# google/hdrnet

Measured on NVIDIA H100. Metric: megapixels/s BilateralSliceApply @4K, higher is better.
Workload: dtype f32

## Files before the change

### hdrnet_b200/csrc/common.cuh

```cuda
#pragma once

#include <cuda_runtime.h>
#include <stdint.h>

#include "hdrnet_b200.h"

namespace hdrnet_b200 {

struct SliceGeom {
  int B;
  int H;
  int W;
  int rows;
  int y_off;
  int gh, gw, gd;
  float scale_x;
  float scale_y;
};

__host__ inline SliceGeom make_geom(int B, int H, int W, int rows, int y_off, int gh, int gw,
                                    int gd) {
  SliceGeom g;
  g.B = B; g.H = H; g.W = W; g.rows = rows; g.y_off = y_off;
  g.gh = gh; g.gw = gw; g.gd = gd;
// ... 131 lines not shown
               "r"(smem_u32(smem_src)), "r"(bytes)
               : "memory");
}
__device__ __forceinline__ void tma_store_commit() {
  asm volatile("cp.async.bulk.commit_group;" ::: "memory");
}
template <int N>
__device__ __forceinline__ void tma_store_wait_read() {
  asm volatile("cp.async.bulk.wait_group.read %0;" ::"n"(N) : "memory");
}
template <int N>
__device__ __forceinline__ void tma_store_wait_all() {
  asm volatile("cp.async.bulk.wait_group %0;" ::"n"(N) : "memory");
}
__device__ __forceinline__ void l2_prefetch_bulk(const void* gmem_src, uint32_t bytes) {
  asm volatile("cp.async.bulk.prefetch.L2.global [%0], %1;" ::"l"(gmem_src), "r"(bytes) : "memory");
}
__device__ __forceinline__ void fence_proxy_async_smem() {
  asm volatile("fence.proxy.async.shared::cta;" ::: "memory");
}

__device__ __forceinline__ uint64_t l2_policy_evict_first() {
  uint64_t p;
  asm volatile("createpolicy.fractional.L2::evict_first.b64 %0, 1.0;" : "=l"(p));
  return p;
}
__device__ __forceinline__ uint64_t l2_policy_evict_last() {
  uint64_t p;
  asm volatile("createpolicy.fractional.L2::evict_last.b64 %0, 1.0;" : "=l"(p));
  return p;
}
__device__ __forceinline__ void tma_load_1d(void* smem_dst, const void* gmem_src, uint32_t bytes,
                                            uint64_t* bar, uint64_t policy) {
  asm volatile(
      "cp.async.bulk.shared::cluster.global.mbarrier::complete_tx::bytes.L2::cache_hint"
      " [%0], [%1], %2, [%3], %4;"
      ::"r"(smem_u32(smem_dst)), "l"(gmem_src), "r"(bytes), "r"(smem_u32(bar)), "l"(policy)
      : "memory");
}
__device__ __forceinline__ void tma_store_1d(void* gmem_dst, const void* smem_src, uint32_t bytes,
                                             uint64_t policy) {
  asm volatile("cp.async.bulk.global.shared::cta.bulk_group.L2::cache_hint [%0], [%1], %2, %3;"
               ::"l"(gmem_dst), "r"(smem_u32(smem_src)), "r"(bytes), "l"(policy)
               : "memory");
}
__device__ __forceinline__ void st_global_hint(float4* p, const float4& v, uint64_t policy) {
  asm volatile("st.global.L2::cache_hint.v4.f32 [%0], {%1, %2, %3, %4}, %5;"
               ::"l"(p), "f"(v.x), "f"(v.y), "f"(v.z), "f"(v.w), "l"(policy)
               : "memory");
}
__device__ __forceinline__ void l2_discard_line(const void* p) {
  asm volatile("discard.global.L2 [%0], 128;" ::"l"(p) : "memory");
}

}
```

### hdrnet_b200/csrc/slice_apply.cu

```cuda
#include <cuda_runtime.h>

#include <atomic>

#include <algorithm>
#include <climits>
#include <cstdint>
#include <cstdlib>
#include <mutex>
#include <new>
#include <vector>

#include "slice_rows.cuh"

namespace hdrnet_b200 {


template <bool kApply>
__global__ void __launch_bounds__(256)
slice_generic_kernel(const float* __restrict__ grid, const float* __restrict__ guide,
                     const float* __restrict__ input, float* __restrict__ out, SliceGeom g,
                     int n_in, int n_out, int J, long long npix) {
  const int gc = kApply ? n_out * J : J;
  const long long grid_image = static_cast<long long>(g.gh) * g.gw * g.gd * gc;
  const long long stride = static_cast<long long>(gridDim.x) * blockDim.x;
// ... 602 lines not shown
      ws[static_cast<size_t>(row) * n_out + e] = lerp4(1.0f - ay.f, va, ay.f, vb);
    }
  }
}

static int launch_yblend(const float* grid, float* ws, const SliceGeom& g, int row_floats, cudaStream_t stream) {
  const long long total_rows = static_cast<long long>(g.B) * g.rows;
  const unsigned blocks = static_cast<unsigned>((total_rows + kYblendRows - 1) / kYblendRows);
  yblend_rows_kernel<<<blocks, 256, 0, stream>>>(grid, reinterpret_cast<float4*>(ws), g, row_floats);
  return static_cast<int>(cudaGetLastError());
}


static int device_sm_count() {
  int dev = 0, sms = 0;
  if (cudaGetDevice(&dev) != cudaSuccess) return 132;
  if (cudaDeviceGetAttribute(&sms, cudaDevAttrMultiProcessorCount, dev) != cudaSuccess) return 132;
  return sms > 0 ? sms : 132;
}

static int device_max_smem_optin() {
  int dev = 0, v = 0;
  if (cudaGetDevice(&dev) != cudaSuccess) return 227 * 1024;
  if (cudaDeviceGetAttribute(&v, cudaDevAttrMaxSharedMemoryPerBlockOptin, dev) != cudaSuccess)
    return 227 * 1024;
  return v;
}

static int device_texture_alignment() {
  int dev = 0, v = 0;
  if (cudaGetDevice(&dev) != cudaSuccess) return 512;
  if (cudaDeviceGetAttribute(&v, cudaDevAttrTextureAlignment, dev) != cudaSuccess) return 512;
  return v > 0 ? v : 512;
}


static bool make_tma_plan(const SliceGeom& g, int max_smem, int sms, TmaPlan* out, bool tex_mode,
                          int threads, int in_fmt = kPxF32, int out_fmt = kPxF32, int grid_rows = 0) {
  const int in_bpp = 3 * px_bytes_per_channel(in_fmt), out_bpp = 3 * px_bytes_per_channel(out_fmt);
  const int gran = std::max(4, std::max(16 / std::__gcd(16, in_bpp), 16 / std::__gcd(16, out_bpp)));
  if (g.W < gran || (g.W % gran) != 0) return false;
  TmaPlan p;
  p.threads = threads;
  p.row_floats = g.gw * g.gd * kGc;
  p.in_bpp = in_bpp;
  p.out_bpp = out_bpp;
  const int quads = g.W / 4;
  p.nseg = (quads + threads - 1) / threads;
  p.seg_px = round_up(4 * ((quads + p.nseg - 1) / p.nseg), gran);
  p.off_guide = round_up(p.seg_px * in_bpp, 16);
  p.off_out = (out_bpp == in_bpp) ? 0 : p.off_guide + p.seg_px * 4;
  p.stage_bytes = round_up((p.off_out ? p.off_out + p.seg_px * out_bpp : p.off_guide + p.seg_px * 4), 128);
  p.off_raw = 256;
  p.off_slab = p.off_raw + round_up(2 * p.row_floats * 4, 128);
  p.off_grid = p.off_slab;
  p.off_stage = p.off_slab + (tex_mode ? grid_rows * round_up(p.row_floats * 4, 128) : round_up(p.row_floats * 4, 128));
  const int per_cta_2 = (max_smem + 1024) / 2 - 1024;
  int stages = 0, resident = 0;
  for (int ns = 4; ns >= 2 && stages == 0; --ns)
    if (p.off_stage + ns * p.stage_bytes <= per_cta_2) { stages = ns; resident = 2; }
  for (int ns = 4; ns >= 2 && stages == 0; --ns)
    if (p.off_stage + ns * p.stage_bytes <= max_smem) { stages = ns; resident = 1; }
  if (stages == 0) return false;
  p.stages = stages;
  p.resident = resident;
  p.smem_bytes = p.off_stage + stages * p.stage_bytes;
  const long long total_rows = static_cast<long long>(g.B) * g.rows;
  p.ctas = static_cast<int>(std::min<long long>(total_rows, static_cast<long long>(sms) * resident));
  *out = p;
  return true;
}

static inline bool aligned16(const void* p) { return (reinterpret_cast<uintptr_t>(p) & 15u) == 0; }

static int validate_common(int B, int H, int W, int gh, int gw, int gd) {
  if (B < 0 || H < 0 || W < 0) return HDRNET_E_BAD_SHAPE;
  if (gh < 1 || gw < 1 || gd < 1) return HDRNET_E_BAD_SHAPE;
  return HDRNET_OK;
}

static int generic_grid(long long npix, int sms) {
  const long long blocks = (npix + 255) / 256;
  return static_cast<int>(std::min<long long>(blocks, static_cast<long long>(sms) * 16));
}

template <class GuideFn, int kTexChunks = 0, int kMinBlocks = 2, int kThreads = kTmaThreads,
          int kIn = kPxF32, int kOut = kPxF32>
static int launch_tma_occ(const TmaArgs& a, const GuideFn& fn, cudaStream_t stream) {
  auto kern = slice_apply_rows_tma_kernel<GuideFn, kTexChunks, kMinBlocks, kThreads, kIn, kOut>;
  cudaError_t e = cudaFuncSetAttribute(kern, cudaFuncAttributeMaxDynamicSharedMemorySize,
                                       a.p.smem_bytes);
  if (e != cudaSuccess) return static_cast<int>(e);
  kern<<<a.p.ctas, kThreads, a.p.smem_bytes, stream>>>(a, fn);
  return static_cast<int>(cudaGetLastError());
}

template <class GuideFn, int kTexChunks = 0>
static int launch_tma(const TmaArgs& a, const GuideFn& fn, cudaStream_t stream, int in_fmt = kPxF32,
                      int out_fmt = kPxF32) {
  if constexpr (GuideFn::kFromInput) {
    if constexpr (kTexChunks > 0) return launch_tma_occ<GuideFn, kTexChunks, 2, kTexThreads>(a, fn, stream);
    else return launch_tma_occ<GuideFn, 0, 2>(a, fn, stream);
  } else {
    if (in_fmt == kPxU8 && out_fmt == kPxU8)
      return launch_tma_occ<GuideFn, kTexChunks, 2, kTmaThreads, kPxU8, kPxU8>(a, fn, stream);
    if (in_fmt == kPxU16 && out_fmt == kPxU8)
// ... 113 lines not shown

static int graph_slab_texture(const float* ws, size_t bytes, cudaGraph_t graph, cudaTextureObject_t* out) {
  cudaStreamCaptureMode mode = cudaStreamCaptureModeRelaxed;
  cudaError_t err = cudaThreadExchangeStreamCaptureMode(&mode);
  if (err != cudaSuccess) { (void)cudaGetLastError(); return static_cast<int>(err); }
  const int rc = graph_slab_texture_relaxed(ws, bytes, graph, out);
  cudaThreadExchangeStreamCaptureMode(&mode);
  return rc;
}

struct GuideSpec {
  int mode;
  const float* guide;
  float* guide_out;
  const CurvesGuideParams* curves;
  const NNGuideParams* nn;
  float* workspace = nullptr;
  size_t workspace_bytes = 0;
  int in_fmt = kPxF32;
  int out_fmt = kPxF32;
};


template <class GuideFn>
static int launch_px_generic(const float* grid, const void* input, void* out, float* guide_out,
                             const SliceGeom& g, long long npix, int blocks, int in_fmt, int out_fmt,
                             const GuideFn& fn, cudaStream_t stream) {
  const unsigned char* in = static_cast<const unsigned char*>(input);
  unsigned char* o = static_cast<unsigned char*>(out);
#define HDRNET_PX_CASE(I, O)                                                                    \
  if (in_fmt == I && out_fmt == O) {                                                            \
    slice_apply_px_generic_kernel<GuideFn, I, O><<<blocks, 256, 0, stream>>>(grid, in, o,       \
                                                                           guide_out, g, npix, fn); \
    return static_cast<int>(cudaGetLastError());                                                \
  }
  HDRNET_PX_CASE(kPxU8, kPxU8)
  HDRNET_PX_CASE(kPxU16, kPxU8)
  HDRNET_PX_CASE(kPxF32, kPxU8)
  HDRNET_PX_CASE(kPxU8, kPxF32)
  HDRNET_PX_CASE(kPxU16, kPxF32)
  HDRNET_PX_CASE(kPxU8, kPxU16)
  HDRNET_PX_CASE(kPxU16, kPxU16)
  HDRNET_PX_CASE(kPxF32, kPxU16)
#undef HDRNET_PX_CASE
  return HDRNET_E_UNSUPPORTED;
}

struct ApplyForm {
  int variant;
  TmaPlan p;
  bool pre_pass;
  bool slab_warp;
  bool lean;
  bool fused_async;
  bool rows_any;
  int ctas, threads;
  size_t smem_bytes;
};

static int plan_slice_apply(const SliceGeom& g, int n_in, int n_out, int has_offset, int mode, int in_fmt,
                            int out_fmt, bool aligned, uintptr_t ws_base, size_t ws_bytes, int variant,
                            ApplyForm* f) {
  const int sms = device_sm_count();
  const int max_smem = device_max_smem_optin();
  const bool px = in_fmt != kPxF32 || out_fmt != kPxF32;
  const long long npix = static_cast<long long>(g.B) * g.rows * g.W;
  *f = ApplyForm{};

  TmaPlan plan;
  const bool row_shape = n_in == 3 && n_out == 3 && has_offset && aligned &&
                         (!px || (in_fmt != kPxF32 && (out_fmt == kPxU8 || out_fmt == kPxU16))) &&
                         make_tma_plan(g, max_smem, sms, &plan, false, kTmaThreads, in_fmt, out_fmt);
  const bool tex_ok = row_shape && ws_base != 0 && ws_base % device_texture_alignment() == 0 &&
                      ws_bytes >= static_cast<size_t>(g.B) * g.rows * plan.row_floats * sizeof(float) &&
                      ws_bytes / 16 <= (1u << 27);
  TmaPlan aplan, splan;
  const bool async_ok = tex_ok && mode == 0 && !px &&
                        make_tma_plan(g, max_smem, sms, &aplan, true, kAsyncThreads - 32) &&
                        aplan.resident == 2 && aplan.seg_px <= aplan.threads * 4;
  const bool slab_lines = (static_cast<size_t>(plan.row_floats) * sizeof(float)) % 128 == 0 && ws_base % 128 == 0;
  const bool slab_warp = async_ok && slab_lines &&
                         make_tma_plan(g, max_smem, sms, &splan, true, kAsyncThreads - 32, kPxF32, kPxF32, 2) &&
                         splan.resident == 2 && splan.seg_px <= splan.threads * 4 &&
                         splan.stages >= kAsyncAutoMinStages;

  const bool auto_req = variant == HDRNET_VARIANT_AUTO;
  if (auto_req) {
    if (tex_ok && g.W >= 128 && npix >= (1LL << 21))
      variant = (async_ok && aplan.stages >= kAsyncAutoMinStages) ? HDRNET_VARIANT_TEX_ASYNC : HDRNET_VARIANT_TEX;
    else
      variant = (row_shape && g.W >= 128) ? HDRNET_VARIANT_TMA : HDRNET_VARIANT_GENERIC;
  }
  f->variant = variant;

  if (variant == HDRNET_VARIANT_GENERIC) {
    if (mode != 0 && !px) return HDRNET_E_UNSUPPORTED;
    const int J = n_in + (has_offset ? 1 : 0);
    const AnyArgs aa{nullptr, nullptr, nullptr, nullptr, g, n_in, n_out, J, n_out * J, g.gw * g.gd * n_out * J};
    const size_t smem = (auto_req && mode == 0) ? rows_any_smem(aa, true, max_smem) : 0;
    f->rows_any = smem != 0;
    f->ctas = f->rows_any ? rows_any_ctas(g, sms) : generic_grid(npix, sms);
    f->threads = f->rows_any ? kAnyThreads : 256;
    f->smem_bytes = smem;
    return HDRNET_OK;
  }
  if (variant == HDRNET_VARIANT_TMA) {
    if (!row_shape) return HDRNET_E_UNSUPPORTED;
    f->p = plan;
  } else if (variant == HDRNET_VARIANT_TEX_ASYNC) {
    if (!async_ok) return HDRNET_E_UNSUPPORTED;
    f->slab_warp = slab_warp;
    f->pre_pass = !slab_warp;
    f->lean = static_cast<long long>(g.W) >= 4LL * g.gw;
    f->p = slab_warp ? splan : aplan;
  } else {
    if (!tex_ok) return HDRNET_E_UNSUPPORTED;
    f->pre_pass = true;
    TmaPlan fplan;
    f->fused_async = mode == 1 &&
                     make_tma_plan(g, max_smem, sms, &fplan, true, kFusedAsyncMathThreads, in_fmt, out_fmt) &&
                     fplan.resident == kFusedAsyncResident && fplan.stages >= 3;
    if (f->fused_async) {
      f->p = fplan;
    } else if (!make_tma_plan(g, max_smem, sms, &f->p, true, mode != 0 ? kTmaThreads : kTexThreads, in_fmt, out_fmt)) {
      return HDRNET_E_UNSUPPORTED;
    }
  }
  const bool issuer = variant == HDRNET_VARIANT_TEX_ASYNC || f->fused_async;
  f->ctas = f->p.ctas;
  f->threads = f->p.threads + (issuer ? 32 : 0) + (f->slab_warp ? 32 : 0);
  f->smem_bytes = f->p.smem_bytes;
  return HDRNET_OK;
}

template <int kTexChunks>
static int launch_block_sync(const TmaArgs& a, const GuideSpec& gs, cudaStream_t stream) {
  if (gs.mode == 1) { GuideCurves fn; fn.p = *gs.curves; return launch_tma<GuideCurves, kTexChunks>(a, fn, stream, gs.in_fmt, gs.out_fmt); }
  if (gs.mode == 2 && gs.nn->feats <= 16) {
    GuideNN<16> fn; fn.p = *gs.nn;
    return launch_tma<GuideNN<16>, kTexChunks>(a, fn, stream, gs.in_fmt, gs.out_fmt);
  }
  if (gs.mode == 2) {
    GuideNN<kMaxGuideFeats> fn; fn.p = *gs.nn;
    return launch_tma<GuideNN<kMaxGuideFeats>, kTexChunks>(a, fn, stream, gs.in_fmt, gs.out_fmt);
  }
  return launch_tma<GuideFromInput, kTexChunks>(a, GuideFromInput{}, stream);
}

static int launch_slice_apply_impl(const float* grid, const GuideSpec& gs, const void* input_v,
                                   void* out_v, int B, int H, int W, int rows, int y_off, int gh,
                                   int gw, int gd, int n_in, int n_out, int has_offset,
                                   int variant, cudaStream_t stream) {
  const float* input = static_cast<const float*>(input_v);
  float* out = static_cast<float*>(out_v);
  const bool px = gs.in_fmt != kPxF32 || gs.out_fmt != kPxF32;
  if (px) {
    if (gs.mode == 0 || n_in != 3 || n_out != 3 || !has_offset) return HDRNET_E_UNSUPPORTED;
    if (gs.in_fmt < kPxF32 || gs.in_fmt > kPxU16 || gs.out_fmt < kPxF32 || gs.out_fmt > kPxU16)
      return HDRNET_E_UNSUPPORTED;
  }
  int rc = validate_common(B, H, W, gh, gw, gd);
  if (rc != HDRNET_OK) return rc;
  if (n_in < 1 || n_out < 1 || rows < 0 || y_off < 0 || y_off + rows > H) return HDRNET_E_BAD_SHAPE;
  const long long npix = static_cast<long long>(B) * rows * W;
  if (npix == 0) return HDRNET_OK;
  if (!grid || !input || !out || (gs.mode == 0 && !gs.guide)) return HDRNET_E_NULL_POINTER;
  if (gs.out_fmt == kPxU16) {
    const uintptr_t o0 = reinterpret_cast<uintptr_t>(out_v), o1 = o0 + static_cast<uintptr_t>(npix) * 6u;
    const uintptr_t i0 = reinterpret_cast<uintptr_t>(input_v),
                    i1 = i0 + static_cast<uintptr_t>(npix) * 3u * px_bytes_per_channel(gs.in_fmt);
    const uintptr_t g0 = reinterpret_cast<uintptr_t>(grid),
                    g1 = g0 + static_cast<uintptr_t>(B) * gh * gw * gd * kGc * sizeof(float);
    if ((o0 < i1 && i0 < o1) || (o0 < g1 && g0 < o1)) return HDRNET_E_UNSUPPORTED;
  }
  const int J = n_in + (has_offset ? 1 : 0);
  const long long grid_floats = static_cast<long long>(gh) * gw * gd * n_out * J;
  if (grid_floats > INT_MAX || static_cast<long long>(rows) * B > INT_MAX / 4) return HDRNET_E_TOO_LARGE;
  if (variant != HDRNET_VARIANT_AUTO && variant != HDRNET_VARIANT_GENERIC && variant != HDRNET_VARIANT_TMA &&
      variant != HDRNET_VARIANT_TEX && variant != HDRNET_VARIANT_TEX_ASYNC)
    return HDRNET_E_UNSUPPORTED;

  const SliceGeom g = make_geom(B, H, W, rows, y_off, gh, gw, gd);
  const bool aligned = aligned16(grid) && aligned16(input) && aligned16(out) &&
                       (gs.mode != 0 || aligned16(gs.guide)) && (gs.guide_out == nullptr || aligned16(gs.guide_out));
  ApplyForm f;
  rc = plan_slice_apply(g, n_in, n_out, has_offset, gs.mode, gs.in_fmt, gs.out_fmt, aligned,
                        reinterpret_cast<uintptr_t>(gs.workspace), gs.workspace_bytes, variant, &f);
  if (rc != HDRNET_OK) return rc;

  if (f.variant == HDRNET_VARIANT_GENERIC) {
    if (px) {
      if (gs.mode == 1) { GuideCurves fn; fn.p = *gs.curves;
                          return launch_px_generic(grid, input_v, out_v, gs.guide_out, g, npix, f.ctas, gs.in_fmt, gs.out_fmt, fn, stream); }
      if (gs.nn->feats <= 16) { GuideNN<16> fn; fn.p = *gs.nn;
                                return launch_px_generic(grid, input_v, out_v, gs.guide_out, g, npix, f.ctas, gs.in_fmt, gs.out_fmt, fn, stream); }
      GuideNN<kMaxGuideFeats> fn; fn.p = *gs.nn;
      return launch_px_generic(grid, input_v, out_v, gs.guide_out, g, npix, f.ctas, gs.in_fmt, gs.out_fmt, fn, stream);
    }
    if (f.rows_any) {
      const AnyArgs aa{grid, gs.guide, input, out, g, n_in, n_out, J, n_out * J, gw * gd * n_out * J};
      return launch_rows_any<true>(aa, f.ctas, f.smem_bytes, device_max_smem_optin(), stream);
    }
    slice_generic_kernel<true><<<f.ctas, 256, 0, stream>>>(grid, gs.guide, input, out, g, n_in, n_out, J, npix);
    return static_cast<int>(cudaGetLastError());
  }

  TmaArgs a;
  a.grid = grid; a.guide = gs.guide; a.guide_out = gs.guide_out;
  a.input = static_cast<const unsigned char*>(input_v); a.out = static_cast<unsigned char*>(out_v);
  a.g = g; a.p = f.p; a.slab_tex = 0; a.yslab = nullptr;
  if (f.variant == HDRNET_VARIANT_TMA) return launch_block_sync<0>(a, gs, stream);

  a.yslab = gs.workspace;
  cudaEvent_t tex_use = nullptr;
  cudaStreamCaptureStatus capture = cudaStreamCaptureStatusNone;
  cudaGraph_t graph = nullptr;
  if (cudaStreamGetCaptureInfo(stream, &capture, nullptr, &graph) != cudaSuccess) {
    (void)cudaGetLastError();
    capture = cudaStreamCaptureStatusNone;
  }
  rc = capture == cudaStreamCaptureStatusActive
           ? graph_slab_texture(gs.workspace, gs.workspace_bytes, graph, &a.slab_tex)
           : get_slab_texture(gs.workspace, gs.workspace_bytes, &a.slab_tex, &tex_use);
  if (rc != 0) return rc;
  if (f.pre_pass) {
    rc = launch_yblend(grid, gs.workspace, g, f.p.row_floats, stream);
    if (rc != 0) return rc;
  }
  if (f.variant == HDRNET_VARIANT_TEX_ASYNC) {
    a.guide_out = nullptr;
    rc = launch_async_form(a, f.lean, f.slab_warp, stream);
  } else if (f.fused_async) {
    rc = launch_async_fused(a, *gs.curves, gs.in_fmt, gs.out_fmt, stream);
  } else {
    rc = launch_block_sync<kSyncTexChunks>(a, gs, stream);
  }
  if (rc == 0 && tex_use && cudaEventRecord(tex_use, stream) != cudaSuccess) rc = static_cast<int>(cudaGetLastError());
  return rc;
}

int launch_slice_apply(const float* grid, const float* guide, const float* input, float* out,
                       int B, int H, int W, int rows, int y_off, int gh, int gw, int gd,
                       int n_in, int n_out, int has_offset, int variant, cudaStream_t stream) {
  GuideSpec gs{0, guide, nullptr, nullptr, nullptr};
  return launch_slice_apply_impl(grid, gs, input, out, B, H, W, rows, y_off, gh, gw, gd, n_in,
                                 n_out, has_offset, variant, stream);
}

int pack_curves_params(CurvesGuideParams* p, const float* ccm, const float* ccm_bias,
                       const float* shifts, const float* slopes, const float* mix,
                       float mix_bias);
int pack_nn_params(NNGuideParams* p, const float* w1, const float* b1, const float* w2, float b2,
                   int feats);

int launch_slice(const float* grid, const float* guide, float* out, int B, int H, int W, int rows,
                 int y_off, int gh, int gw, int gd, int gc, int variant, cudaStream_t stream) {
  int rc = validate_common(B, H, W, gh, gw, gd);
  if (rc != HDRNET_OK) return rc;
  if (gc < 1 || rows < 0 || y_off < 0 || y_off + rows > H) return HDRNET_E_BAD_SHAPE;
  const long long npix = static_cast<long long>(B) * rows * W;
  if (npix == 0) return HDRNET_OK;
  if (!grid || !guide || !out) return HDRNET_E_NULL_POINTER;
  if (static_cast<long long>(gh) * gw * gd * gc > INT_MAX) return HDRNET_E_TOO_LARGE;
  if (variant != HDRNET_VARIANT_AUTO && variant != HDRNET_VARIANT_GENERIC &&
      variant != HDRNET_VARIANT_TMA)
    return HDRNET_E_UNSUPPORTED;
  const SliceGeom g = make_geom(B, H, W, rows, y_off, gh, gw, gd);
  const int sms = device_sm_count();
  SlicePlan plan;
  const bool tma_shape = gc == kGc && make_slice_plan(g, device_max_smem_optin(), sms, &plan) &&
                         aligned16(grid) && aligned16(guide) && aligned16(out);
  if (variant == HDRNET_VARIANT_TMA && !tma_shape) return HDRNET_E_UNSUPPORTED;
  const bool use_tma = tma_shape && (variant == HDRNET_VARIANT_TMA ||
                                     (variant == HDRNET_VARIANT_AUTO && W >= 128));
  if (use_tma) {
    cudaError_t e = cudaFuncSetAttribute(slice_rows_tma_kernel,
                                         cudaFuncAttributeMaxDynamicSharedMemorySize,
                                         plan.smem_bytes);
    if (e != cudaSuccess) return static_cast<int>(e);
    SliceArgs a;
    a.grid = grid; a.guide = guide; a.out = out; a.g = g; a.p = plan;
    slice_rows_tma_kernel<<<plan.ctas, kSliceThreads, plan.smem_bytes, stream>>>(a);
  } else {
// ... 1 lines not shown
      const int max_smem = device_max_smem_optin();
      AnyArgs aa{grid, guide, nullptr, out, g, 0, gc, 1, gc, gw * gd * gc};
      const size_t smem = rows_any_smem(aa, false, max_smem);
      if (smem) return launch_rows_any<false>(aa, rows_any_ctas(g, sms), smem, max_smem, stream);
    }
    slice_generic_kernel<false><<<generic_grid(npix, sms), 256, 0, stream>>>(
        grid, guide, nullptr, out, g, 0, 0, gc, npix);
  }
  return static_cast<int>(cudaGetLastError());
}

bool fused_call_runs_row_form(int H, int W, int gh, int gw, int gd, int mode, int in_fmt, int out_fmt,
                              bool aligned) {
  ApplyForm f;
  return plan_slice_apply(make_geom(1, H, W, H, 0, gh, gw, gd), 3, 3, 1, mode, in_fmt, out_fmt, aligned, 0, 0,
                          HDRNET_VARIANT_AUTO, &f) == HDRNET_OK &&
         f.variant != HDRNET_VARIANT_GENERIC;
}

}

using namespace hdrnet_b200;

extern "C" {

int hdrnet_b200_abi_version(void) { return HDRNET_B200_ABI_VERSION; }

const char* hdrnet_b200_error_string(int code) {
  switch (code) {
    case HDRNET_OK: return "ok";
    case HDRNET_E_NULL_POINTER: return "a required pointer is NULL";
    case HDRNET_E_BAD_SHAPE: return "invalid dimension";
    case HDRNET_E_BAD_CHANNELS: return "grid channels do not match n_out * (n_in + has_offset)";
    case HDRNET_E_TOO_LARGE: return "extent exceeds the kernels' 32-bit index range";
    case HDRNET_E_UNSUPPORTED: return "requested kernel variant cannot run these shapes";
    case HDRNET_E_BAD_CONTEXT: return "invalid or destroyed context or model object, or not its device";
    case HDRNET_E_BAD_MODEL: return "malformed frozen model (magic, version, lengths, shapes or CRC-32C)";
    default: break;
  }
  if (code > 0) return cudaGetErrorString(static_cast<cudaError_t>(code));
  return "unknown hdrnet_b200 error";
}

int hdrnet_slice_apply_f32_variant(const float* grid, const float* guide, const float* input,
                                   float* out, int B, int H, int W, int gh, int gw, int gd,
                                   int n_in, int n_out, int has_offset, int variant,
                                   void* stream) {
  return launch_slice_apply(grid, guide, input, out, B, H, W, H, 0, gh, gw, gd, n_in, n_out,
                            has_offset, variant, static_cast<cudaStream_t>(stream));
}

size_t hdrnet_slice_apply_workspace_bytes(int B, int H, int gw, int gd) {
  if (B < 0 || H < 0 || gw < 1 || gd < 1) return 0;
  return static_cast<size_t>(B) * H * gw * gd * kGc * sizeof(float);
}

int hdrnet_slice_apply_f32_ws(const float* grid, const float* guide, const float* input,
                              float* out, int B, int H, int W, int gh, int gw, int gd, int n_in,
                              int n_out, int has_offset, int variant, void* workspace,
                              size_t workspace_bytes, void* stream) {
  GuideSpec gs{0, guide, nullptr, nullptr, nullptr};
  gs.workspace = static_cast<float*>(workspace);
  gs.workspace_bytes = workspace_bytes;
  return launch_slice_apply_impl(grid, gs, input, out, B, H, W, H, 0, gh, gw, gd, n_in, n_out,
                                 has_offset, variant, static_cast<cudaStream_t>(stream));
}

int hdrnet_slice_apply_rows_f32_ws(const float* grid, const float* guide, const float* input,
                                   float* out, int B, int H, int W, int rows, int y_off, int gh,
                                   int gw, int gd, int n_in, int n_out, int has_offset, int variant,
                                   void* workspace, size_t workspace_bytes, void* stream) {
  GuideSpec gs{0, guide, nullptr, nullptr, nullptr};
  gs.workspace = static_cast<float*>(workspace);
  gs.workspace_bytes = workspace_bytes;
  return launch_slice_apply_impl(grid, gs, input, out, B, H, W, rows, y_off, gh, gw, gd, n_in, n_out,
                                 has_offset, variant, static_cast<cudaStream_t>(stream));
}

int hdrnet_slice_apply_f32(const float* grid, const float* guide, const float* input,
                           float* out, int B, int H, int W, int gh, int gw, int gd, int n_in,
                           int n_out, int has_offset, void* stream) {
  return launch_slice_apply(grid, guide, input, out, B, H, W, H, 0, gh, gw, gd, n_in, n_out,
                            has_offset, HDRNET_VARIANT_AUTO, static_cast<cudaStream_t>(stream));
}

extern "C" int hdrnet_guide_curves_f32(const float*, float*, long long, const float*, const float*,
                                       const float*, const float*, const float*, float, void*);
extern "C" int hdrnet_guide_nn_f32(const float*, float*, long long, const float*, const float*,
                                   const float*, float, int, void*);

int hdrnet_slice_apply_curves_f32_ws(const float* grid, const float* input, float* out,
                                     float* guide_out, int B, int H, int W, int gh, int gw, int gd,
                                     const float* ccm, const float* ccm_bias, const float* shifts,
                                     const float* slopes, const float* mix, float mix_bias,
                                     void* workspace, size_t workspace_bytes, void* stream) {
  CurvesGuideParams cp;
  int rc = pack_curves_params(&cp, ccm, ccm_bias, shifts, slopes, mix, mix_bias);
  if (rc != HDRNET_OK) return rc;
  GuideSpec gs{1, nullptr, guide_out, &cp, nullptr};
  gs.workspace = static_cast<float*>(workspace);
  gs.workspace_bytes = workspace_bytes;
  rc = launch_slice_apply_impl(grid, gs, input, out, B, H, W, H, 0, gh, gw, gd, 3, 3, 1,
                               HDRNET_VARIANT_AUTO, static_cast<cudaStream_t>(stream));
  if (rc != HDRNET_E_UNSUPPORTED) return rc;
  if (!guide_out) return HDRNET_E_NULL_POINTER;
  rc = hdrnet_guide_curves_f32(input, guide_out, static_cast<long long>(B) * H * W, ccm, ccm_bias,
                               shifts, slopes, mix, mix_bias, stream);
// ... 139 lines not shown
```

### hdrnet_b200/csrc/slice_apply_async.cu

```cuda
#include <cuda_runtime.h>

#include <climits>
#include <cstdint>
#include <cstdlib>

#include "slice_rows.cuh"

namespace hdrnet_b200 {


template <int kTexChunks>
__host__ __device__ constexpr bool chunk_on_tex(int c, int p) { return c * 3 + p >= 12 - kTexChunks; }

template <int kTexChunks, int kC, int kP>
__device__ __forceinline__ ulonglong2 fetch_chunk(const unsigned char* __restrict__ slab_b,
                                                  cudaTextureObject_t tex, int off_b, int tex_idx) {
  if constexpr (chunk_on_tex<kTexChunks>(kC, kP)) {
    const float4 v = tex1Dfetch<float4>(tex, tex_idx + kP);
    ulonglong2 r;
    r.x = pack2(v.x, v.y);
    r.y = pack2(v.z, v.w);
    return r;
  } else {
    return *reinterpret_cast<const ulonglong2*>(slab_b + off_b + 16 * kP);
// ... 105 lines not shown
    *reinterpret_cast<float4*>(args.guide_out + pix) = make_float4(gv[0], gv[1], gv[2], gv[3]);
  }
  const float xf = static_cast<float>(x0 + 4 * q);
  float tx[4];
#pragma unroll
  for (int i = 0; i < 4; ++i)
    tx[i] = __fsub_rn(__fmul_rn(__fadd_rn(xf, static_cast<float>(i) + 0.5f), g.scale_x), 0.5f);
  const int ix0 = __float2int_rd(tx[0]);
  const float fl0 = static_cast<float>(ix0), fl1 = fl0 + 1.0f;
  const int b0 = clampi(ix0, 0, g.gw - 1) * g.gd * 48;
  const int b1 = clampi(ix0 + 1, 0, g.gw - 1) * g.gd * 48;
  const int b2 = clampi(ix0 + 2, 0, g.gw - 1) * g.gd * 48;
  float o_r[4], o_g[4], o_b[4];
#pragma unroll
  for (int i = 0; i < 4; ++i) {
    const bool step = (i > 0) && (tx[i] >= fl1);
    const float fx = tx[i] - (step ? fl1 : fl0);
    const int xo0 = step ? b1 : b0;
    const int xo1 = step ? b2 : b1;
    const float tz = __fsub_rn(__fmul_rn(gv[i], gd_f), 0.5f);
    const int iz = __float2int_rd(tz);
    const float fz = tz - static_cast<float>(iz);
    const int zc0 = clampi(iz, 0, g.gd - 1);
    const int zc1 = clampi(iz + 1, 0, g.gd - 1);
    float wz0, wz1;
    smoothed_weights(fz, wz0, wz1);
    const float wx1 = fx, wx0 = 1.0f - fx;
    const int off[4] = {zc0 * 48 + xo0, zc1 * 48 + xo0, zc0 * 48 + xo1, zc1 * 48 + xo1};
    int tix[4];
#pragma unroll
    for (int c = 0; c < 4; ++c) tix[c] = tex_base + (off[c] >> 4);
    const float w[4] = {wx0 * wz0, wx0 * wz1, wx1 * wz0, wx1 * wz1};
    blend_apply_q<kTexChunks>(slab_b, args.slab_tex, off, tix, w, pr[i], pg[i], pb[i], o_r[i], o_g[i], o_b[i]);
  }
  store_quad<kOut>(out_tile, q, o_r, o_g, o_b);
  fence_proxy_async_smem();
}

template <int kTexChunks, bool kLean, int kThreads, int kMinBlocks, bool kSlabWarp>
__global__ void __launch_bounds__(kThreads, kMinBlocks)
slice_apply_rows_async_kernel(const TmaArgs args) {
  static_assert(kTexChunks > 0, "the issuer-warp kernel serves part of the gather by texture");
  constexpr int kMathWarps = kThreads / 32 - 1 - (kSlabWarp ? 1 : 0);
  extern __shared__ __align__(128) unsigned char smem[];
  const SliceGeom& g = args.g;
  const TmaPlan& pl = args.p;
  const int tid = threadIdx.x, warp = tid >> 5, lane = tid & 31;

  uint64_t* full = reinterpret_cast<uint64_t*>(smem);
  uint64_t* done = full + kMaxStages;
  uint64_t* slab_full = done + kMaxStages;
  uint64_t* row_free = slab_full + 2;
  uint64_t* grid_full = row_free + 2;
  unsigned char* raw0 = smem + pl.off_raw;
  unsigned char* stage_base = smem + pl.off_stage;

  const long long total_items = static_cast<long long>(g.B) * g.rows * pl.nseg;
  const long long i_begin = total_items * blockIdx.x / gridDim.x;
  const long long i_end = total_items * (blockIdx.x + 1) / gridDim.x;
  if (i_end <= i_begin) return;
  const long long r_begin = i_begin / pl.nseg, r_end = (i_end - 1) / pl.nseg + 1;
  const int x_first = static_cast<int>(i_begin - r_begin * pl.nseg) * pl.seg_px;
  const int x_last = min(g.W, (static_cast<int>((i_end - 1) - (r_end - 1) * pl.nseg) + 1) * pl.seg_px);
  auto row_x0 = [&](long long row) { return row == r_begin ? x_first : 0; };
  auto row_x1 = [&](long long row) { return row == r_end - 1 ? x_last : g.W; };

  if (tid == 0) {
    for (int s = 0; s < pl.stages; ++s) { mbar_init(&full[s], 1); mbar_init(&done[s], kMathWarps); }
    for (int i = 0; i < 2; ++i) { mbar_init(&slab_full[i], 1); mbar_init(&row_free[i], 1); mbar_init(&grid_full[i], 1); }
    fence_mbar_init();
  }
  __syncthreads();

  const int NS = pl.stages;
  const uint32_t slab_bytes = static_cast<uint32_t>(pl.row_floats) * 4u;
  auto arrive = [&](uint64_t* bar) {
    asm volatile("mbarrier.arrive.shared::cta.b64 _, [%0];" ::"r"(smem_u32(bar)) : "memory");
  };

  if (kSlabWarp && warp == kMathWarps + 1) {
    float* graw = reinterpret_cast<float*>(smem + pl.off_grid);
    const int gstride = (static_cast<int>(slab_bytes) + 127) / 128 * 32;
    int key0 = -1, key1 = -1;
    uint32_t gpar0 = 0u, gpar1 = 0u;
    const int n4 = pl.row_floats / 4;
    float4* ws4 = reinterpret_cast<float4*>(const_cast<float*>(args.yslab));
    const uint64_t ws_pol = l2_policy_evict_last();
    auto discard_row = [&](long long r) {
      if (row_x0(r) != 0 || row_x1(r) != g.W) return;
      const unsigned char* base = reinterpret_cast<const unsigned char*>(ws4 + static_cast<size_t>(r) * n4);
      for (int l = lane; l < static_cast<int>(slab_bytes / 128u); l += 32) l2_discard_line(base + 128 * l);
    };
    for (long long row = r_begin; row < r_end; ++row) {
      const int rowk = static_cast<int>(row - r_begin), rb = rowk & 1;
      const int b = static_cast<int>(row / g.rows);
      const int y = g.y_off + static_cast<int>(row - static_cast<long long>(b) * g.rows);
      const Axis ay = spatial_axis(y, g.scale_y);
      const int k0 = b * g.gh + clampi(ay.i0, 0, g.gh - 1);
      const int k1 = b * g.gh + clampi(ay.i0 + 1, 0, g.gh - 1);
      int s0 = (key0 == k0) ? 0 : ((key1 == k0) ? 1 : -1);
      int s1 = (key0 == k1) ? 0 : ((key1 == k1) ? 1 : -1);
      auto fetch = [&](int slot, int k) {
        if (lane == 0) {
          mbar_expect_tx(&grid_full[slot], slab_bytes);
          tma_load_1d(graw + slot * gstride, args.grid + static_cast<size_t>(k) * pl.row_floats, slab_bytes,
                      &grid_full[slot]);
        }
        if (slot == 0) { key0 = k; mbar_wait(&grid_full[0], gpar0); gpar0 ^= 1u; }
        else { key1 = k; mbar_wait(&grid_full[1], gpar1); gpar1 ^= 1u; }
      };
      __syncwarp();
      if (s0 < 0) { s0 = (s1 == 0) ? 1 : 0; fetch(s0, k0); if (k1 == k0) s1 = s0; }
      if (s1 < 0) { s1 = s0 ^ 1; fetch(s1, k1); }
      if (rowk >= 2) mbar_wait(&row_free[rb], static_cast<uint32_t>((rowk >> 1) - 1) & 1u);
      const float wy1 = ay.f, wy0 = 1.0f - ay.f;
      const float4* a4 = reinterpret_cast<const float4*>(graw + s0 * gstride);
      const float4* b4 = reinterpret_cast<const float4*>(graw + s1 * gstride);
      float4* slab4 = reinterpret_cast<float4*>(raw0 + static_cast<size_t>(rb) * slab_bytes);
      float4* wrow = ws4 + static_cast<size_t>(row) * n4;
      for (int e = lane; e < n4; e += 32) {
        const float4 v = lerp4(wy0, a4[e], wy1, b4[e]);
        slab4[e] = v;
        st_global_hint(wrow + e, v, ws_pol);
      }
      __threadfence();
      __syncwarp();
      if (lane == 0) arrive(&slab_full[rb]);
      if (rowk >= 2) discard_row(row - 2);
    }
    for (long long row = max(r_begin, r_end - 2); row < r_end; ++row) {
      const int rowk = static_cast<int>(row - r_begin);
      mbar_wait(&row_free[rowk & 1], static_cast<uint32_t>(rowk >> 1) & 1u);
      discard_row(row);
    }
    return;
  }

  if (warp == kMathWarps) {
    if (lane != 0) return;
    const uint64_t px_pol = l2_policy_evict_first();
    auto make_slab = [&](long long row) {
      if constexpr (kSlabWarp) return;
      const int rb = static_cast<int>(row - r_begin) & 1;
      mbar_expect_tx(&slab_full[rb], slab_bytes);
      tma_load_1d(raw0 + static_cast<size_t>(rb) * slab_bytes,
                  args.yslab + static_cast<size_t>(row) * pl.row_floats, slab_bytes, &slab_full[rb]);
    };
    long long l_row = r_begin;
    int l_x0 = x_first, l_s = 0;
    auto issue_next_load = [&]() {
      if (l_row >= r_end) return;
      const int npx = min(pl.seg_px, g.W - l_x0);
      unsigned char* st = stage_base + static_cast<size_t>(l_s) * pl.stage_bytes;
      const size_t pix = static_cast<size_t>(l_row) * g.W + l_x0;
      mbar_expect_tx(&full[l_s], static_cast<uint32_t>(npx) * 16u);
      tma_load_1d(st, args.input + pix * 12, static_cast<uint32_t>(npx) * 12u, &full[l_s], px_pol);
      tma_load_1d(st + pl.off_guide, args.guide + pix, static_cast<uint32_t>(npx) * 4u, &full[l_s], px_pol);
      if (++l_s == NS) l_s = 0;
      l_x0 += pl.seg_px;
      if (l_x0 >= row_x1(l_row)) { l_x0 = 0; ++l_row; }
    };
    for (int i = 0; i < NS - 1; ++i) issue_next_load();
    make_slab(r_begin);
    if (r_begin + 1 < r_end) make_slab(r_begin + 1);

    int s = 0;
    uint32_t ph = 0;
    for (long long row = r_begin; row < r_end; ++row) {
      const int x_end = row_x1(row);
      for (int x0 = row_x0(row); x0 < x_end; x0 += pl.seg_px) {
        mbar_wait(&done[s], ph);
        const int npx = min(pl.seg_px, g.W - x0);
        unsigned char* st = stage_base + static_cast<size_t>(s) * pl.stage_bytes;
        const size_t pix = static_cast<size_t>(row) * g.W + x0;
        tma_store_1d(args.out + pix * 12, st, static_cast<uint32_t>(npx) * 12u, px_pol);
        tma_store_commit();
        if (l_row < r_end) {
          tma_store_wait_read<1>();
          issue_next_load();
        }
        if (++s == NS) { s = 0; ph ^= 1u; }
      }
      if constexpr (kSlabWarp) arrive(&row_free[static_cast<int>(row - r_begin) & 1]);
      else if (row + 2 < r_end) make_slab(row + 2);
    }
    tma_store_wait_all<0>();
    return;
  }

  const int q = warp * 32 + lane;
  const int cells = g.gw * g.gd;
  int s = 0;
  uint32_t ph = 0;
  for (long long row = r_begin; row < r_end; ++row) {
    const int rowk = static_cast<int>(row - r_begin), rb = rowk & 1;
    mbar_wait(&slab_full[rb], static_cast<uint32_t>(rowk >> 1) & 1u);
    const unsigned char* slab_b = raw0 + static_cast<size_t>(rb) * slab_bytes;
    const int tex_base = static_cast<int>(row) * cells * 3;
    const int x_end = row_x1(row);
    for (int x0 = row_x0(row); x0 < x_end; x0 += pl.seg_px) {
      const int npx = min(pl.seg_px, g.W - x0);
      unsigned char* st = stage_base + static_cast<size_t>(s) * pl.stage_bytes;
      mbar_wait(&full[s], ph);
      if (q * 4 < npx) {
        if constexpr (kLean)
          process_quad_lean<kTexChunks>(args, st, st, st + pl.off_guide, slab_b, tex_base, x0, q);
        else
          process_quad<GuideFromInput, kTexChunks>(args, GuideFromInput{}, st, st, st + pl.off_guide,
                                                   reinterpret_cast<const float*>(slab_b), tex_base,
                                                   row, x0, q);
      }
      __syncwarp();
      if (lane == 0) arrive(&done[s]);
      if (++s == NS) { s = 0; ph ^= 1u; }
    }
  }
}

template <bool kLean, bool kSlabWarp>
static int launch_async(const TmaArgs& a, cudaStream_t stream) {
  constexpr int kLaunchThreads = kAsyncThreads + (kSlabWarp ? 32 : 0);
  auto kern = slice_apply_rows_async_kernel<kAsyncTexChunks, kLean, kLaunchThreads, 2, kSlabWarp>;
  cudaError_t e = cudaFuncSetAttribute(kern, cudaFuncAttributeMaxDynamicSharedMemorySize, a.p.smem_bytes);
  if (e != cudaSuccess) return static_cast<int>(e);
  kern<<<a.p.ctas, kLaunchThreads, a.p.smem_bytes, stream>>>(a);
  return static_cast<int>(cudaGetLastError());
}

int launch_async_form(const TmaArgs& a, bool lean, bool slab_warp, cudaStream_t stream) {
  if (slab_warp) return lean ? launch_async<true, true>(a, stream) : launch_async<false, true>(a, stream);
  return lean ? launch_async<true, false>(a, stream) : launch_async<false, false>(a, stream);
}

constexpr int kFusedAsyncThreads = kFusedAsyncMathThreads + 32;

template <class GuideFn, int kTexChunks, int kIn, int kOut>
__global__ void __launch_bounds__(kFusedAsyncThreads, kFusedAsyncResident)
slice_apply_rows_async_fused_kernel(const TmaArgs args, const __grid_constant__ GuideFn guide_fn) {
  static_assert(!GuideFn::kFromInput, "fused-guide forms only");
  constexpr int kMathWarps = kFusedAsyncThreads / 32 - 1;
  constexpr uint32_t kInBpp = 3u * px_bytes_per_channel(kIn), kOutBpp = 3u * px_bytes_per_channel(kOut);
  extern __shared__ __align__(128) unsigned char smem[];
  const SliceGeom& g = args.g;
  const TmaPlan& pl = args.p;
  const int tid = threadIdx.x, warp = tid >> 5, lane = tid & 31;

  uint64_t* full = reinterpret_cast<uint64_t*>(smem);
  uint64_t* done = full + kMaxStages;
  uint64_t* slab_full = done + kMaxStages;
  unsigned char* raw0 = smem + pl.off_raw;
  unsigned char* stage_base = smem + pl.off_stage;

  const long long total_items = static_cast<long long>(g.B) * g.rows * pl.nseg;
// ... 116 lines not shown
```

### hdrnet_b200/csrc/slice_rows.cuh

```cuda
#pragma once

#include <cuda_runtime.h>

#include <cstdint>

#include "common.cuh"
#include "guide.cuh"

namespace hdrnet_b200 {

constexpr int kPxF32 = HDRNET_PX_F32, kPxU8 = HDRNET_PX_U8, kPxU16 = HDRNET_PX_U16;

__host__ __device__ constexpr int px_bytes_per_channel(int fmt) {
  return fmt == kPxU8 ? 1 : (fmt == kPxU16 ? 2 : 4);
}

template <int kFmt>
__device__ __forceinline__ float px_to_float(unsigned v) {
  constexpr float D = (kFmt == kPxU8) ? 255.0f : 65535.0f;
  constexpr float R = 1.0f / D;
  const float f = static_cast<float>(v);
  const float q0 = f * R;
  return fmaf(fmaf(-q0, D, f), R, q0);
}
// ... 41 lines not shown
                                           const float (&o_g)[4], const float (&o_b)[4]) {
  if constexpr (kFmt == kPxF32) {
    float4* rgb4 = reinterpret_cast<float4*>(tile) + 3 * q;
    rgb4[0] = make_float4(o_r[0], o_g[0], o_b[0], o_r[1]);
    rgb4[1] = make_float4(o_g[1], o_b[1], o_r[2], o_g[2]);
    rgb4[2] = make_float4(o_b[2], o_r[3], o_g[3], o_b[3]);
  } else if constexpr (kFmt == kPxU8) {
    uint32_t* w = reinterpret_cast<uint32_t*>(tile) + 3 * q;
    w[0] = float_to_u8(o_r[0]) | (float_to_u8(o_g[0]) << 8) | (float_to_u8(o_b[0]) << 16) | (float_to_u8(o_r[1]) << 24);
    w[1] = float_to_u8(o_g[1]) | (float_to_u8(o_b[1]) << 8) | (float_to_u8(o_r[2]) << 16) | (float_to_u8(o_g[2]) << 24);
    w[2] = float_to_u8(o_b[2]) | (float_to_u8(o_r[3]) << 8) | (float_to_u8(o_g[3]) << 16) | (float_to_u8(o_b[3]) << 24);
  } else {
    static_assert(kFmt == kPxU16, "results leave as float32, uint8 or uint16");
    uint2* w = reinterpret_cast<uint2*>(tile) + 3 * q;
    w[0] = make_uint2(float_to_u16(o_r[0]) | (float_to_u16(o_g[0]) << 16), float_to_u16(o_b[0]) | (float_to_u16(o_r[1]) << 16));
    w[1] = make_uint2(float_to_u16(o_g[1]) | (float_to_u16(o_b[1]) << 16), float_to_u16(o_r[2]) | (float_to_u16(o_g[2]) << 16));
    w[2] = make_uint2(float_to_u16(o_b[2]) | (float_to_u16(o_r[3]) << 16), float_to_u16(o_g[3]) | (float_to_u16(o_b[3]) << 16));
  }
}

template <int kFmt>
__device__ __forceinline__ float load_channel(const unsigned char* base, long long idx) {
  if constexpr (kFmt == kPxF32) return __ldg(reinterpret_cast<const float*>(base) + idx);
  else if constexpr (kFmt == kPxU8) return px_to_float<kPxU8>(__ldg(base + idx));
  else return px_to_float<kPxU16>(__ldg(reinterpret_cast<const unsigned short*>(base) + idx));
}


constexpr int kTmaThreads = 256;
constexpr int kTexThreads = 512;
constexpr int kAsyncThreads = 352;
constexpr int kAsyncAutoMinStages = 3;
constexpr int kAsyncTexChunks = 5;
constexpr int kMaxStages = 8;
constexpr int kSyncTexChunks = 4;
constexpr int kGc = 12;

static inline int round_up(int v, int m) { return (v + m - 1) / m * m; }

struct TmaPlan {
  int ctas;
  int threads;
  int resident;
  int stages;
  int nseg;
  int seg_px;
  int row_floats;
  int smem_bytes;
  int off_raw, off_slab, off_stage, stage_bytes;
  int off_grid;
  int in_bpp, out_bpp, off_guide, off_out;
};

struct TmaArgs {
  const float* grid;
  const float* guide;
  float* guide_out;
  const unsigned char* input;
  unsigned char* out;
  cudaTextureObject_t slab_tex;
  const float* yslab;
  SliceGeom g;
  TmaPlan p;
};

__device__ __forceinline__ float4 lerp4(float w0, float4 a, float w1, float4 b) {
  return make_float4(fmaf(w1, b.x, w0 * a.x), fmaf(w1, b.y, w0 * a.y), fmaf(w1, b.z, w0 * a.z),
                     fmaf(w1, b.w, w0 * a.w));
}

template <int kTexChunks, int kChunkId, bool kBytes = false>
__device__ __forceinline__ ulonglong2 corner_chunk(const float* __restrict__ slab,
                                                   cudaTextureObject_t tex, int tex_row, int off) {
  if constexpr (kChunkId >= 12 - kTexChunks) {
    const float4 v = tex1Dfetch<float4>(tex, tex_row + (off >> (kBytes ? 4 : 2)) + (kChunkId % 3));
    ulonglong2 r;
    r.x = pack2(v.x, v.y);
    r.y = pack2(v.z, v.w);
    return r;
  } else if constexpr (kBytes) {
    return reinterpret_cast<const ulonglong2*>(reinterpret_cast<const unsigned char*>(slab) + off)[kChunkId % 3];
  } else {
    return reinterpret_cast<const ulonglong2*>(slab + off)[kChunkId % 3];
  }
}

template <int kTexChunks, bool kBytes = false>
__device__ __forceinline__ void blend_apply(const float* __restrict__ slab,
                                            cudaTextureObject_t tex, int tex_row, int o00,
                                            int o01, int o10, int o11, float w00, float w01,
                                            float w10, float w11, float r, float g, float b,
                                            float& out_r, float& out_g, float& out_b) {
  const unsigned long long W00 = pack2(w00, w00), W01 = pack2(w01, w01);
  const unsigned long long W10 = pack2(w10, w10), W11 = pack2(w11, w11);
  const ulonglong2 a0 = corner_chunk<kTexChunks, 0, kBytes>(slab, tex, tex_row, o00);
  const ulonglong2 a1 = corner_chunk<kTexChunks, 1, kBytes>(slab, tex, tex_row, o00);
  const ulonglong2 a2 = corner_chunk<kTexChunks, 2, kBytes>(slab, tex, tex_row, o00);
  const ulonglong2 b0 = corner_chunk<kTexChunks, 3, kBytes>(slab, tex, tex_row, o01);
  const ulonglong2 b1 = corner_chunk<kTexChunks, 4, kBytes>(slab, tex, tex_row, o01);
  const ulonglong2 b2 = corner_chunk<kTexChunks, 5, kBytes>(slab, tex, tex_row, o01);
  const ulonglong2 c0 = corner_chunk<kTexChunks, 6, kBytes>(slab, tex, tex_row, o10);
  const ulonglong2 c1 = corner_chunk<kTexChunks, 7, kBytes>(slab, tex, tex_row, o10);
  const ulonglong2 c2 = corner_chunk<kTexChunks, 8, kBytes>(slab, tex, tex_row, o10);
  const ulonglong2 d0 = corner_chunk<kTexChunks, 9, kBytes>(slab, tex, tex_row, o11);
  const ulonglong2 d1 = corner_chunk<kTexChunks, 10, kBytes>(slab, tex, tex_row, o11);
  const ulonglong2 d2 = corner_chunk<kTexChunks, 11, kBytes>(slab, tex, tex_row, o11);
  unsigned long long acc[6];
  acc[0] = fma2(W11, d0.x, fma2(W10, c0.x, fma2(W01, b0.x, mul2(W00, a0.x))));
  acc[1] = fma2(W11, d0.y, fma2(W10, c0.y, fma2(W01, b0.y, mul2(W00, a0.y))));
  acc[2] = fma2(W11, d1.x, fma2(W10, c1.x, fma2(W01, b1.x, mul2(W00, a1.x))));
  acc[3] = fma2(W11, d1.y, fma2(W10, c1.y, fma2(W01, b1.y, mul2(W00, a1.y))));
  acc[4] = fma2(W11, d2.x, fma2(W10, c2.x, fma2(W01, b2.x, mul2(W00, a2.x))));
  acc[5] = fma2(W11, d2.y, fma2(W10, c2.y, fma2(W01, b2.y, mul2(W00, a2.y))));
  float a0f, a1f, a2f, a3f;
  unpack2(acc[0], a0f, a1f);
  unpack2(acc[1], a2f, a3f);
// ... 181 lines not shown
```

Baseline: 96960.

## Add dynamic tail row scheduling via global atomic work queue in async slice kernel

Each CTA statically processes a fixed number of rows (kStaticRows per CTA). The remaining rows are pulled dynamically from a global atomic counter stored in a workspace tail region, guarded by a per-launch nonce. Row indices are communicated from the producer thread to the slab and math warps through a small shared-memory ring, and each loop now ends on a -1 sentinel. The aim is to balance load and reduce tail imbalance across CTAs. The cost is atomic traffic, a spin-wait on the nonce, extra workspace bytes, and the path being disabled under graph capture.

```diff
diff --git a/hdrnet_b200/csrc/common.cuh b/hdrnet_b200/csrc/common.cuh
--- a/hdrnet_b200/csrc/common.cuh
+++ b/hdrnet_b200/csrc/common.cuh
@@ -207,5 +207,10 @@
 __device__ __forceinline__ void l2_discard_line(const void* p) {
   asm volatile("discard.global.L2 [%0], 128;" ::"l"(p) : "memory");
 }
-
-}
+__device__ __forceinline__ unsigned long long ld_acquire_gpu(const unsigned long long* p) {
+  unsigned long long v;
+  asm volatile("ld.acquire.gpu.global.u64 %0, [%1];" : "=l"(v) : "l"(p) : "memory");
+  return v;
+}
+
+}
diff --git a/hdrnet_b200/csrc/slice_apply.cu b/hdrnet_b200/csrc/slice_apply.cu
--- a/hdrnet_b200/csrc/slice_apply.cu
+++ b/hdrnet_b200/csrc/slice_apply.cu
@@ -678,6 +678,7 @@
   p.off_out = (out_bpp == in_bpp) ? 0 : p.off_guide + p.seg_px * 4;
   p.stage_bytes = round_up((p.off_out ? p.off_out + p.seg_px * out_bpp : p.off_guide + p.seg_px * 4), 128);
   p.off_raw = 256;
+  static_assert((2 * kMaxStages + 6) * 8 + kRowSlots * 4 <= 256, "barrier region");
   p.off_slab = p.off_raw + round_up(2 * p.row_floats * 4, 128);
   p.off_grid = p.off_slab;
   p.off_stage = p.off_slab + (tex_mode ? grid_rows * round_up(p.row_floats * 4, 128) : round_up(p.row_floats * 4, 128));
@@ -897,6 +898,7 @@
   bool pre_pass;
   bool slab_warp;
   bool lean;
+  long long tail_row0;
   bool fused_async;
   bool rows_any;
   int ctas, threads;
@@ -958,6 +960,11 @@
     f->pre_pass = !slab_warp;
     f->lean = static_cast<long long>(g.W) >= 4LL * g.gw;
     f->p = slab_warp ? splan : aplan;
+    const long long nrows = static_cast<long long>(g.B) * g.rows;
+    const long long row0 = static_cast<long long>(kStaticRows) * f->p.ctas;
+    const bool tail = row0 < nrows &&
+                      ws_bytes >= static_cast<size_t>(nrows) * plan.row_floats * sizeof(float) + kSliceTailBytes;
+    f->tail_row0 = tail ? row0 : nrows;
   } else {
     if (!tex_ok) return HDRNET_E_UNSUPPORTED;
     f->pre_pass = true;
@@ -1054,6 +1061,7 @@
   a.grid = grid; a.guide = gs.guide; a.guide_out = gs.guide_out;
   a.input = static_cast<const unsigned char*>(input_v); a.out = static_cast<unsigned char*>(out_v);
   a.g = g; a.p = f.p; a.slab_tex = 0; a.yslab = nullptr;
+  a.tail = nullptr; a.nonce = 0; a.tail_row0 = static_cast<long long>(B) * rows;
   if (f.variant == HDRNET_VARIANT_TMA) return launch_block_sync<0>(a, gs, stream);
 
   a.yslab = gs.workspace;
@@ -1074,6 +1082,13 @@
   }
   if (f.variant == HDRNET_VARIANT_TEX_ASYNC) {
     a.guide_out = nullptr;
+    if (f.tail_row0 < a.tail_row0 && capture != cudaStreamCaptureStatusActive) {
+      static std::atomic<unsigned long long> next_nonce{1};
+      a.tail = reinterpret_cast<SliceTail*>(reinterpret_cast<unsigned char*>(gs.workspace) +
+                                            static_cast<size_t>(a.tail_row0) * f.p.row_floats * sizeof(float));
+      a.nonce = next_nonce.fetch_add(1, std::memory_order_relaxed);
+      a.tail_row0 = f.tail_row0;
+    }
     rc = launch_async_form(a, f.lean, f.slab_warp, stream);
   } else if (f.fused_async) {
     rc = launch_async_fused(a, *gs.curves, gs.in_fmt, gs.out_fmt, stream);
@@ -1181,7 +1196,7 @@
 
 size_t hdrnet_slice_apply_workspace_bytes(int B, int H, int gw, int gd) {
   if (B < 0 || H < 0 || gw < 1 || gd < 1) return 0;
-  return static_cast<size_t>(B) * H * gw * gd * kGc * sizeof(float);
+  return static_cast<size_t>(B) * H * gw * gd * kGc * sizeof(float) + kSliceTailBytes;
 }
 
 int hdrnet_slice_apply_f32_ws(const float* grid, const float* guide, const float* input,
diff --git a/hdrnet_b200/csrc/slice_apply_async.cu b/hdrnet_b200/csrc/slice_apply_async.cu
--- a/hdrnet_b200/csrc/slice_apply_async.cu
+++ b/hdrnet_b200/csrc/slice_apply_async.cu
@@ -181,25 +181,36 @@
   uint64_t* slab_full = done + kMaxStages;
   uint64_t* row_free = slab_full + 2;
   uint64_t* grid_full = row_free + 2;
+  int* row_slot = reinterpret_cast<int*>(grid_full + 2);
   unsigned char* raw0 = smem + pl.off_raw;
   unsigned char* stage_base = smem + pl.off_stage;
 
-  const long long total_items = static_cast<long long>(g.B) * g.rows * pl.nseg;
+  SliceTail* const tail = args.tail;
+  if (tail != nullptr && blockIdx.x == 0 && tid == 0) {
+    *reinterpret_cast<volatile unsigned int*>(&tail->next) = 0u;
+    __threadfence();
+    *reinterpret_cast<volatile unsigned long long*>(&tail->nonce) = args.nonce;
+  }
+  const long long total_items = args.tail_row0 * pl.nseg;
   const long long i_begin = total_items * blockIdx.x / gridDim.x;
   const long long i_end = total_items * (blockIdx.x + 1) / gridDim.x;
   if (i_end <= i_begin) return;
-  const long long r_begin = i_begin / pl.nseg, r_end = (i_end - 1) / pl.nseg + 1;
-  const int x_first = static_cast<int>(i_begin - r_begin * pl.nseg) * pl.seg_px;
-  const int x_last = min(g.W, (static_cast<int>((i_end - 1) - (r_end - 1) * pl.nseg) + 1) * pl.seg_px);
-  auto row_x0 = [&](long long row) { return row == r_begin ? x_first : 0; };
-  auto row_x1 = [&](long long row) { return row == r_end - 1 ? x_last : g.W; };
-
   if (tid == 0) {
     for (int s = 0; s < pl.stages; ++s) { mbar_init(&full[s], 1); mbar_init(&done[s], kMathWarps); }
     for (int i = 0; i < 2; ++i) { mbar_init(&slab_full[i], 1); mbar_init(&row_free[i], 1); mbar_init(&grid_full[i], 1); }
     fence_mbar_init();
   }
   __syncthreads();
+
+  const int r_begin = static_cast<int>(i_begin / pl.nseg), r_end = static_cast<int>((i_end - 1) / pl.nseg + 1);
+  const int nstat = r_end - r_begin;
+  const int x_first = static_cast<int>(i_begin - static_cast<long long>(r_begin) * pl.nseg) * pl.seg_px;
+  const int x_last = min(g.W, (static_cast<int>((i_end - 1) - static_cast<long long>(r_end - 1) * pl.nseg) + 1) * pl.seg_px);
+  auto row_x0 = [&](int row) { return row == r_begin ? x_first : 0; };
+  auto row_x1 = [&](int row) { return row == r_end - 1 ? x_last : g.W; };
+  auto local_row = [&](int k) -> int {
+    return k < nstat ? r_begin + k : (tail != nullptr ? row_slot[k % kRowSlots] : -1);
+  };
 
   const int NS = pl.stages;
   const uint32_t slab_bytes = static_cast<uint32_t>(pl.row_floats) * 4u;
@@ -215,15 +226,24 @@
     const int n4 = pl.row_floats / 4;
     float4* ws4 = reinterpret_cast<float4*>(const_cast<float*>(args.yslab));
     const uint64_t ws_pol = l2_policy_evict_last();
-    auto discard_row = [&](long long r) {
+    auto discard_row = [&](int r) {
       if (row_x0(r) != 0 || row_x1(r) != g.W) return;
       const unsigned char* base = reinterpret_cast<const unsigned char*>(ws4 + static_cast<size_t>(r) * n4);
       for (int l = lane; l < static_cast<int>(slab_bytes / 128u); l += 32) l2_discard_line(base + 128 * l);
     };
-    for (long long row = r_begin; row < r_end; ++row) {
-      const int rowk = static_cast<int>(row - r_begin), rb = rowk & 1;
-      const int b = static_cast<int>(row / g.rows);
-      const int y = g.y_off + static_cast<int>(row - static_cast<long long>(b) * g.rows);
+    int row_m1 = -1, row_m2 = -1;
+    int rowk = 0;
+    for (;; ++rowk) {
+      const int rb = rowk & 1;
+      if (rowk >= 2) mbar_wait(&row_free[rb], static_cast<uint32_t>((rowk >> 1) - 1) & 1u);
+      const int row = local_row(rowk);
+      if (row < 0) {
+        __syncwarp();
+        if (lane == 0) arrive(&slab_full[rb]);
+        break;
+      }
+      const int b = row / g.rows;
+      const int y = g.y_off + (row - b * g.rows);
       const Axis ay = spatial_axis(y, g.scale_y);
       const int k0 = b * g.gh + clampi(ay.i0, 0, g.gh - 1);
       const int k1 = b * g.gh + clampi(ay.i0 + 1, 0, g.gh - 1);
@@ -241,7 +261,6 @@
       __syncwarp();
       if (s0 < 0) { s0 = (s1 == 0) ? 1 : 0; fetch(s0, k0); if (k1 == k0) s1 = s0; }
       if (s1 < 0) { s1 = s0 ^ 1; fetch(s1, k1); }
-      if (rowk >= 2) mbar_wait(&row_free[rb], static_cast<uint32_t>((rowk >> 1) - 1) & 1u);
       const float wy1 = ay.f, wy0 = 1.0f - ay.f;
       const float4* a4 = reinterpret_cast<const float4*>(graw + s0 * gstride);
       const float4* b4 = reinterpret_cast<const float4*>(graw + s1 * gstride);
@@ -255,12 +274,13 @@
       __threadfence();
       __syncwarp();
       if (lane == 0) arrive(&slab_full[rb]);
-      if (rowk >= 2) discard_row(row - 2);
+      if (rowk >= 2) discard_row(row_m2);
+      row_m2 = row_m1;
+      row_m1 = row;
     }
-    for (long long row = max(r_begin, r_end - 2); row < r_end; ++row) {
-      const int rowk = static_cast<int>(row - r_begin);
-      mbar_wait(&row_free[rowk & 1], static_cast<uint32_t>(rowk >> 1) & 1u);
-      discard_row(row);
+    for (int k = max(0, rowk - 2); k < rowk; ++k) {
+      mbar_wait(&row_free[k & 1], static_cast<uint32_t>(k >> 1) & 1u);
+      discard_row(k == rowk - 1 ? row_m1 : row_m2);
     }
     return;
   }
@@ -268,17 +288,40 @@
   if (warp == kMathWarps) {
     if (lane != 0) return;
     const uint64_t px_pol = l2_policy_evict_first();
-    auto make_slab = [&](long long row) {
+    int k_taken = nstat;
+    bool pool_open = tail != nullptr, nonce_seen = false;
+    auto row_at = [&](int k) -> int {
+      if (k < nstat) return r_begin + k;
+      while (k_taken <= k && pool_open) {
+        if (!nonce_seen) {
+          while (ld_acquire_gpu(&tail->nonce) != args.nonce) {}
+          nonce_seen = true;
+        }
+        const long long r = args.tail_row0 + atomicAdd(&tail->next, 1u);
+        pool_open = r < static_cast<long long>(g.B) * g.rows;
+        row_slot[k_taken++ % kRowSlots] = pool_open ? static_cast<int>(r) : -1;
+      }
+      return k < k_taken ? row_slot[k % kRowSlots] : -1;
+    };
+    bool end_sent = false;
+    auto make_slab = [&](int k) {
       if constexpr (kSlabWarp) return;
-      const int rb = static_cast<int>(row - r_begin) & 1;
+      const int rb = k & 1;
+      const int row = row_at(k);
+      if (row < 0) {
+        if (!end_sent) arrive(&slab_full[rb]);
+        end_sent = true;
+        return;
+      }
       mbar_expect_tx(&slab_full[rb], slab_bytes);
       tma_load_1d(raw0 + static_cast<size_t>(rb) * slab_bytes,
                   args.yslab + static_cast<size_t>(row) * pl.row_floats, slab_bytes, &slab_full[rb]);
     };
-    long long l_row = r_begin;
+    int l_k = 0;
+    int l_row = r_begin;
     int l_x0 = x_first, l_s = 0;
     auto issue_next_load = [&]() {
-      if (l_row >= r_end) return;
+      if (l_row < 0) return;
       const int npx = min(pl.seg_px, g.W - l_x0);
       unsigned char* st = stage_base + static_cast<size_t>(l_s) * pl.stage_bytes;
       const size_t pix = static_cast<size_t>(l_row) * g.W + l_x0;
@@ -287,15 +330,17 @@
       tma_load_1d(st + pl.off_guide, args.guide + pix, static_cast<uint32_t>(npx) * 4u, &full[l_s], px_pol);
       if (++l_s == NS) l_s = 0;
       l_x0 += pl.seg_px;
-      if (l_x0 >= row_x1(l_row)) { l_x0 = 0; ++l_row; }
+      if (l_x0 >= row_x1(l_row)) { l_x0 = 0; l_row = row_at(++l_k); }
     };
     for (int i = 0; i < NS - 1; ++i) issue_next_load();
-    make_slab(r_begin);
-    if (r_begin + 1 < r_end) make_slab(r_begin + 1);
+    make_slab(0);
+    make_slab(1);
 
     int s = 0;
     uint32_t ph = 0;
-    for (long long row = r_begin; row < r_end; ++row) {
+    for (int k = 0;; ++k) {
+      const int row = row_at(k);
+      if (row < 0) break;
       const int x_end = row_x1(row);
       for (int x0 = row_x0(row); x0 < x_end; x0 += pl.seg_px) {
         mbar_wait(&done[s], ph);
@@ -304,14 +349,18 @@
         const size_t pix = static_cast<size_t>(row) * g.W + x0;
         tma_store_1d(args.out + pix * 12, st, static_cast<uint32_t>(npx) * 12u, px_pol);
         tma_store_commit();
-        if (l_row < r_end) {
+        if (l_row >= 0) {
           tma_store_wait_read<1>();
           issue_next_load();
         }
         if (++s == NS) { s = 0; ph ^= 1u; }
       }
-      if constexpr (kSlabWarp) arrive(&row_free[static_cast<int>(row - r_begin) & 1]);
-      else if (row + 2 < r_end) make_slab(row + 2);
+      if constexpr (kSlabWarp) {
+        (void)row_at(k + 2);
+        arrive(&row_free[k & 1]);
+      } else {
+        make_slab(k + 2);
+      }
     }
     tma_store_wait_all<0>();
     return;
@@ -321,13 +370,15 @@
   const int cells = g.gw * g.gd;
   int s = 0;
   uint32_t ph = 0;
-  for (long long row = r_begin; row < r_end; ++row) {
-    const int rowk = static_cast<int>(row - r_begin), rb = rowk & 1;
+  for (int rowk = 0;; ++rowk) {
+    const int rb = rowk & 1;
     mbar_wait(&slab_full[rb], static_cast<uint32_t>(rowk >> 1) & 1u);
+    const int row = local_row(rowk);
+    if (row < 0) break;
     const unsigned char* slab_b = raw0 + static_cast<size_t>(rb) * slab_bytes;
-    const int tex_base = static_cast<int>(row) * cells * 3;
-    const int x_end = row_x1(row);
-    for (int x0 = row_x0(row); x0 < x_end; x0 += pl.seg_px) {
+    const int tex_base = row * cells * 3;
+    const int x_end = rowk == nstat - 1 ? x_last : g.W;
+    for (int x0 = rowk == 0 ? x_first : 0; x0 < x_end; x0 += pl.seg_px) {
       const int npx = min(pl.seg_px, g.W - x0);
       unsigned char* st = stage_base + static_cast<size_t>(s) * pl.stage_bytes;
       mbar_wait(&full[s], ph);
diff --git a/hdrnet_b200/csrc/slice_rows.cuh b/hdrnet_b200/csrc/slice_rows.cuh
--- a/hdrnet_b200/csrc/slice_rows.cuh
+++ b/hdrnet_b200/csrc/slice_rows.cuh
@@ -117,6 +117,15 @@
   int in_bpp, out_bpp, off_guide, off_out;
 };
 
+constexpr int kStaticRows = 2;
+constexpr int kSliceTailBytes = 128;
+constexpr int kRowSlots = 8;
+struct SliceTail {
+  unsigned int next;
+  unsigned int pad;
+  unsigned long long nonce;
+};
+
 struct TmaArgs {
   const float* grid;
   const float* guide;
@@ -127,6 +136,9 @@
   const float* yslab;
   SliceGeom g;
   TmaPlan p;
+  SliceTail* tail;
+  unsigned long long nonce;
+  long long tail_row0;
 };
 
 __device__ __forceinline__ float4 lerp4(float w0, float4 a, float w1, float4 b) {
```

Measured after the change: 104,100 (median of 6 runs). 7.4% higher.
